# Circuitscape/Circuitscape.jl

Measured on NVIDIA H100. Metric: pair_solves_per_sec, higher is better.
Workload: dtype f64

## Files before the change

### circuitscape_b200/csrc/cs_b200.cu

```cuda
#include "../../include/cs_b200.h"

#include <cuda_runtime.h>

#include <algorithm>
#include <chrono>
#include <cmath>
#include <cstdarg>
#include <cstdio>
#include <cstdlib>
#include <cstring>
#include <limits>
#include <string>
#include <vector>

#include "amg_host.hpp"
#include "win_host.hpp"
#include "kernels.cuh"
#include "raster_assembly.cuh"
#include "setup_device.hpp"

using namespace csb;

namespace {

thread_local std::string g_create_error;

struct GraphSlot {
  cudaGraphExec_t exec = nullptr;
  int chunk = 0;
  int64_t kernels = 0, spmms = 0;
  cudaGraphExec_t loop_exec = nullptr;
  int64_t loop_kernels = 0, loop_spmms = 0;
};

}

struct DevCsr {
  int* rowptr = nullptr;
  int* colidx = nullptr;
  void* vals = nullptr;
  int* bstart = nullptr;
  int nblocks = 0;
  int nrows = 0;
  int64_t nnz = 0;
  int lpr = 1;
  WinMeta* win_meta = nullptr;
  unsigned char* blob = nullptr;
  int has_dinv = 0;
// ... 10 lines not shown
struct DevLevel {
  int64_t n = 0, n_pad = 0;
  DevCsr A, P, R;
  void* dinv = nullptr;
  double omega = 2.0 / 3.0;
  void *x = nullptr, *b = nullptr, *t = nullptr, *y = nullptr;
};

struct cs_b200_handle {
  int device = 0;
  int dtype = CS_B200_F64;
  int64_t n = 0, n_pad = 0, nnz = 0;
  int* d_rowptr = nullptr;
  int* d_colidx = nullptr;
  void* d_vals = nullptr;
  bool owns_matrix = true;
  void* d_vals0 = nullptr;
  void* d_dinv = nullptr;
  int* d_bstart = nullptr;
  int nblocks = 0;
  int ktmax = 8;
  void *X = nullptr, *R = nullptr, *P = nullptr, *AP = nullptr, *B = nullptr, *stage = nullptr;
  void* Z = nullptr;
  DevCsr A0;
  std::vector<DevLevel> lv;
  double* d_pinv = nullptr;
  double amg_opc = 0.0;
  bool amg = false;
  bool mixed = false;
  std::vector<DevLevel> lv32;
  void *R32 = nullptr, *X32 = nullptr, *T32 = nullptr, *Z32 = nullptr;
  void *d_cum = nullptr, *d_max = nullptr;
  PanelCtl* d_ctl = nullptr;
  PanelCtl* h_ctl = nullptr;
  double* d_partials = nullptr;
  float* d_flush = nullptr;
  size_t flush_elems = 0;
  cudaStream_t stream = nullptr;
  cudaEvent_t ev0 = nullptr, ev1 = nullptr, ev2 = nullptr, ev3 = nullptr;
  long long* d_sp_rows = nullptr;
  double* d_sp_vals = nullptr;
  int* d_sp_ptr = nullptr;
  size_t sp_cap = 0;
  long long* d_probe = nullptr;
  void* d_probe_out = nullptr;
  size_t probe_cap = 0;
  cudaStream_t s_in = nullptr, s_out = nullptr;
  void* io_in[2] = {nullptr, nullptr};
  void* io_out[2] = {nullptr, nullptr};
  cudaEvent_t ev_in[2] = {nullptr, nullptr}, ev_used[2] = {nullptr, nullptr};
  cudaEvent_t ev_ready[2] = {nullptr, nullptr}, ev_out[2] = {nullptr, nullptr};
  int num_sms = 132;
  int grid_spmm = 132, grid_ew = 132;
  cs_b200_opts opts{};
  cs_b200_stats stats{};
  GraphSlot graphs[4];
  bool rg_on = false;
  int* d_rg_seg = nullptr;
  int* d_rg_rows = nullptr;
  size_t rg_cap = 0;
  GraphSlot rgraphs[4];
  int profile = 0;
  std::vector<cudaEvent_t> prof_ev;
  size_t prof_used = 0;
  double prof_ms = 0.0;
  double prof_bytes = 0.0;
  int64_t prof_launches = 0;
  std::vector<int> prof_slot;
  std::vector<double> prof_pair_bytes;
  double prof_slot_ms[16] = {}, prof_slot_bytes[16] = {};
  int64_t prof_slot_launches[16] = {};
  std::string err;
  size_t esize() const { return dtype == CS_B200_F64 ? 8 : 4; }
};

namespace {

struct Tick {
  bool on = std::getenv("CS_B200_VERBOSE") != nullptr;
  std::chrono::steady_clock::time_point t0 = std::chrono::steady_clock::now();
  void operator()(const char* what) {
    if (!on) return;
    const auto t1 = std::chrono::steady_clock::now();
    std::fprintf(stderr, "[cs_b200 setup] %-28s %8.1f ms\n", what,
                 std::chrono::duration<double, std::milli>(t1 - t0).count());
    t0 = t1;
  }
};

int set_err(cs_b200_handle* h, int code, const char* fmt, ...) {
  char buf[1024];
  va_list ap;
  va_start(ap, fmt);
  vsnprintf(buf, sizeof buf, fmt, ap);
// ... 525 lines not shown
  rc = build_operators<T>(h, hp, job, dseed);
  if (rc) return rc;
  return cs_b200_reset_currents(h);
}

template <typename T>
int build_operators(cs_b200_handle* h, const csb_dev::HostPattern& hp, csb_dev::SeedJob* job,
                    const csb_dev::DeviceSeed* dseed) {
  int rc = CS_B200_OK;
  k_dinv<T><<<std::min<int64_t>((h->n_pad + 255) / 256, 4096), 256, 0, h->stream>>>(
      (int)h->n, (int)h->n_pad, h->d_rowptr, h->d_colidx, (const T*)h->d_vals, (T*)h->d_dinv);
  const bool want_win = h->opts.window >= 0 && (h->opts.window > 0 || h->n >= 20000) && (win_mask() & 1);
  const bool want_amg = h->opts.precond == CS_B200_PRECOND_AMG;
  Tick tick;
  if (want_win || h->opts.stencil > 0) {
    rc = device_stencil<T>(h, h->A0);
    if (!rc && !h->A0.dia && want_win) rc = device_windows<T>(h, h->A0, h->n_pad, (const T*)h->d_dinv);
    if (rc) { csb_dev::seed_discard(job); return rc; }
    tick(h->A0.dia ? "finest operator: stencil form" : "finest operator: windows");
  }
  if (want_amg) {
    rc = setup_amg_device<T>(h, hp, job, dseed);
    if (rc) return rc;
  } else {
    csb_dev::seed_discard(job);
  }
  Tick tick1;
  csb_dev::trim_pool(h->device);
  tick1("scratch pool released");
  return CS_B200_OK;
}

int common_create(cs_b200_handle* h, const cs_b200_opts* opts) {
  if (opts) h->opts = *opts;
  if (h->opts.panel_width == 0) h->opts.panel_width = 8;
  if (h->opts.check_every <= 0) h->opts.check_every = 16;
  if (h->opts.resid_gate <= 0) h->opts.resid_gate = 1e-4;
  if (h->opts.use_graph == 0) h->opts.use_graph = 1;
  const int pw = h->opts.panel_width;
  if (pw != 1 && pw != 2 && pw != 4 && pw != 8)
    return set_err(h, CS_B200_ERR_ARG, "panel_width must be 1, 2, 4 or 8 (got %d)", pw);
  h->ktmax = pw;
  if (h->opts.precond != CS_B200_PRECOND_JACOBI && h->opts.precond != CS_B200_PRECOND_AMG)
    return set_err(h, CS_B200_ERR_UNSUPPORTED, "unknown preconditioner %d", h->opts.precond);
  int ndev = 0;
  cudaError_t e = cudaGetDeviceCount(&ndev);
// ... 84 lines not shown
    }
  } else if (m.lpr == 4 && KT * 4 <= 32) {
    k_spmm<T, KT, MODE, (KT * 4 <= 32 ? 4 : 1)><<<grid, NT, 0, h->stream>>>(view<T>(m), X, Y, ep);
  } else {
    k_spmm<T, KT, MODE, 1><<<grid, NT, 0, h->stream>>>(view<T>(m), X, Y, ep);
  }
  if (prof) cudaEventRecord(e1, h->stream);
  h->stats.kernel_launches++;
  if (timed) h->stats.spmm_launches++;
}

template <typename T, int KT, int MODE>
void launch_spmm(cs_b200_handle* h, const T* X, T* Y, const T* B) {
  launch_spmm_on<T, KT, MODE>(h, h->A0, X, Y, B, (const T*)h->d_dinv, 0.0, true);
}

void harvest_profile(cs_b200_handle* h) {
  for (size_t i = 0; i + 1 < h->prof_used; i += 2) {
    float ms = 0;
    if (cudaEventElapsedTime(&ms, h->prof_ev[i], h->prof_ev[i + 1]) == cudaSuccess) {
      h->prof_ms += ms;
      h->prof_launches++;
      if (i / 2 < h->prof_slot.size()) {
        const int sl = h->prof_slot[i / 2] & 15;
        h->prof_slot_ms[sl] += ms;
        h->prof_slot_bytes[sl] += h->prof_pair_bytes[i / 2];
        h->prof_slot_launches[sl]++;
      }
    }
  }
  h->prof_used = 0;
  h->prof_slot.clear();
  h->prof_pair_bytes.clear();
}

template <typename T, int KT>
int ew_grid(cs_b200_handle* h) {
  const size_t nelem = (size_t)h->n_pad * KT;
  const size_t per = (size_t)NT * Vec<T>::N;
  return (int)std::min<size_t>(h->grid_ew, (nelem + per - 1) / per);
}

template <typename T, int KT>
int ew_grid_n(cs_b200_handle* h, int64_t n_pad) {
  const size_t nelem = (size_t)n_pad * KT;
  const size_t per = (size_t)NT * Vec<T>::N;
  return (int)std::max<size_t>(1, std::min<size_t>(h->grid_ew, (nelem + per - 1) / per));
// ... 143 lines not shown
  k_seg_set<T, KT><<<2 * KT, NT, 0, h->stream>>>((T*)panel, h->d_rg_seg, h->d_rg_rows, set_b_only, v);
  h->stats.kernel_launches++;
}

template <typename T, int KT>
void mask_z(cs_b200_handle* h) {
  if (!h->rg_on) return;
  if (h->mixed) launch_seg_set<float, KT>(h, h->Z32, 0, 0.0f);
  else launch_seg_set<T, KT>(h, h->Z, 0, T(0));
}

inline GraphSlot& graph_slot(cs_b200_handle* h, int kt) {
  return (h->rg_on ? h->rgraphs : h->graphs)[kt_index(kt)];
}

void drop_graphs(GraphSlot* slots) {
  for (int i = 0; i < 4; ++i) {
    if (slots[i].exec) cudaGraphExecDestroy(slots[i].exec);
    if (slots[i].loop_exec) cudaGraphExecDestroy(slots[i].loop_exec);
    slots[i] = GraphSlot{};
  }
}

template <typename T, int KT>
void launch_iteration(cs_b200_handle* h) {
  const size_t nelem = (size_t)h->n_pad * KT;
  const int g = ew_grid<T, KT>(h);
  launch_spmm<T, KT, SP_CG>(h, (const T*)h->P, (T*)h->AP, nullptr);
  if (h->rg_on) launch_seg_set<T, KT>(h, h->AP, 0, T(0));
  if (!h->amg) {
    k_cg_update_r<T, KT><<<g, NT, 0, h->stream>>>(nelem, (const T*)h->AP, (const T*)h->d_dinv,
                                                  (T*)h->R, h->d_ctl, h->d_partials);
    k_cg_update_xp<T, KT><<<g, NT, 0, h->stream>>>(nelem, (const T*)h->R, (const T*)h->d_dinv,
                                                   (T*)h->X, (T*)h->P, h->d_ctl);
    h->stats.kernel_launches += 2;
  } else {
    if (h->mixed) {
      k_cg_update_r0<T, KT, float><<<g, NT, 0, h->stream>>>(nelem, (const T*)h->AP, (const T*)h->d_dinv,
                                                            (T)h->lv[0].omega, (T*)h->R,
                                                            implicit_x0(h->lv32[0]) ? nullptr : (float*)h->X32,
                                                            (float*)h->R32, h->d_ctl);
      launch_vcycle<T, KT>(h, true);
      mask_z<T, KT>(h);
      k_cg_update_xp2<T, KT, float><<<g, NT, 0, h->stream>>>(nelem, (const float*)h->Z32, (T*)h->X, (T*)h->P,
                                                             h->d_ctl);
    } else {
      k_cg_update_r0<T, KT, T><<<g, NT, 0, h->stream>>>(nelem, (const T*)h->AP, (const T*)h->d_dinv,
                                                        (T)h->lv[0].omega, (T*)h->R,
                                                        implicit_x0(h->lv[0]) ? nullptr : (T*)h->stage, nullptr,
                                                        h->d_ctl);
      launch_vcycle<T, KT>(h, true);
      mask_z<T, KT>(h);
      k_cg_update_xp2<T, KT, T><<<g, NT, 0, h->stream>>>(nelem, (const T*)h->Z, (T*)h->X, (T*)h->P, h->d_ctl);
    }
    h->stats.kernel_launches += 2;
  }
}

template <typename T, int KT>
int run_chunk(cs_b200_handle* h, int chunk) {
  GraphSlot& gs = graph_slot(h, KT);
  if (h->opts.use_graph > 0 && !h->profile) {
    if (!gs.exec || gs.chunk != chunk) {
      if (gs.exec) cudaGraphExecDestroy(gs.exec);
      gs.exec = nullptr;
      cudaGraph_t graph;
      const int64_t kl = h->stats.kernel_launches, sl = h->stats.spmm_launches;
      CK(h, cudaStreamBeginCapture(h->stream, cudaStreamCaptureModeThreadLocal));
      for (int i = 0; i < chunk; ++i) launch_iteration<T, KT>(h);
      CK(h, cudaStreamEndCapture(h->stream, &graph));
      gs.kernels = h->stats.kernel_launches - kl;
      gs.spmms = h->stats.spmm_launches - sl;
      h->stats.kernel_launches = kl;
      h->stats.spmm_launches = sl;
      CK(h, cudaGraphInstantiate(&gs.exec, graph, 0));
      cudaGraphDestroy(graph);
      gs.chunk = chunk;
    }
    CK(h, cudaGraphLaunch(gs.exec, h->stream));
// ... 41 lines not shown
    CK(h, cudaGraphInstantiate(&gs.loop_exec, graph, 0));
    cudaGraphDestroy(graph);
  }
  CK(h, cudaGraphLaunch(gs.loop_exec, h->stream));
  return CS_B200_OK;
}

template <typename T, int KT>
int solve_panel(cs_b200_handle* h, double rtol, int64_t itmax) {
  const size_t nelem = (size_t)h->n_pad * KT;
  const double atol = h->opts.atol > 0 ? h->opts.atol
                      : h->opts.atol < 0 ? 0.0
                      : std::sqrt(std::numeric_limits<double>::epsilon());
  const int g = ew_grid<T, KT>(h);
  const int imax = (int)std::min<int64_t>(itmax, std::numeric_limits<int>::max() - 1);
  CK(h, cudaEventRecord(h->ev2, h->stream));
  if (!h->amg) {
    k_set_stall<<<1, 1, 0, h->stream>>>(h->d_ctl, 2000);
    k_cg_init<T, KT><<<g, NT, 0, h->stream>>>(nelem, (const T*)h->B, (const T*)h->d_dinv, (T*)h->X,
                                              (T*)h->R, (T*)h->P, h->d_ctl, h->d_partials, rtol, atol,
                                              imax);
    h->stats.kernel_launches++;
  } else {
    CK(h, cudaMemsetAsync(h->X, 0, nelem * sizeof(T), h->stream));
    CK(h, cudaMemsetAsync(h->P, 0, nelem * sizeof(T), h->stream));
    CK(h, cudaMemcpyAsync(h->R, h->B, nelem * sizeof(T), cudaMemcpyDeviceToDevice, h->stream));
    k_set_ctl<<<1, 1, 0, h->stream>>>(h->d_ctl, rtol, atol, imax, 40);
    if (h->mixed) {
      k_convert<T, float><<<g, NT, 0, h->stream>>>(nelem, (const T*)h->R, (float*)h->R32);
      launch_vcycle<T, KT>(h, false);
      mask_z<T, KT>(h);
      k_cg_update_xp2<T, KT, float><<<g, NT, 0, h->stream>>>(nelem, (const float*)h->Z32, (T*)h->X, (T*)h->P,
                                                             h->d_ctl);
      h->stats.kernel_launches++;
    } else {
      launch_vcycle<T, KT>(h, false);
      mask_z<T, KT>(h);
      k_cg_update_xp2<T, KT, T><<<g, NT, 0, h->stream>>>(nelem, (const T*)h->Z, (T*)h->X, (T*)h->P, h->d_ctl);
    }
    h->stats.kernel_launches += 2;
  }
  CK(h, cudaGetLastError());
  const int chunk = h->amg ? std::min(h->opts.check_every, 4) : h->opts.check_every;
  const bool device_loop = h->opts.use_graph == 1 && !h->profile;
  if (device_loop) {
    int rc = run_loop<T, KT>(h);
    if (rc) return rc;
  }
  for (;;) {
    CK(h, cudaMemcpyAsync(h->h_ctl, h->d_ctl, sizeof(PanelCtl), cudaMemcpyDeviceToHost, h->stream));
    CK(h, cudaStreamSynchronize(h->stream));
    if (h->profile) harvest_profile(h);
    if (device_loop) {
      GraphSlot& gs = graph_slot(h, KT);
      h->stats.kernel_launches += 1 + gs.loop_kernels * h->h_ctl->iter;
      h->stats.spmm_launches += gs.loop_spmms * h->h_ctl->iter;
      break;
    }
    if (h->h_ctl->nactive == 0) break;
    int rc = run_chunk<T, KT>(h, chunk);
    if (rc) return rc;
  }
  if (h->rg_on) {
    launch_spmm<T, KT, SP_RES>(h, (const T*)h->X, (T*)h->AP, (const T*)h->B);
    launch_seg_set<T, KT>(h, h->AP, 0, T(0));
    k_resnorm<T, KT><<<g, NT, 0, h->stream>>>(nelem, (size_t)h->n * KT, (const T*)h->AP, (const T*)h->B, h->d_ctl, h->d_partials);
    h->stats.kernel_launches++;
  } else {
    launch_spmm<T, KT, 2>(h, (const T*)h->X, (T*)h->AP, (const T*)h->B);
  }
  CK(h, cudaGetLastError());
  CK(h, cudaEventRecord(h->ev3, h->stream));
  CK(h, cudaMemcpyAsync(h->h_ctl, h->d_ctl, sizeof(PanelCtl), cudaMemcpyDeviceToHost, h->stream));
  CK(h, cudaStreamSynchronize(h->stream));
  if (h->profile) harvest_profile(h);
  float ms = 0;
  CK(h, cudaEventElapsedTime(&ms, h->ev2, h->ev3));
  h->stats.kernel_ms += ms;
  return CS_B200_OK;
}

int gather_panel_status(cs_b200_handle* h, int kt, int64_t c0, int64_t* iters, double* relres,
                        int64_t itmax, bool* any_fail, bool* any_maxit, std::string* msg) {
  for (int c = 0; c < kt; ++c) {
    const PanelCtl& ct = *h->h_ctl;
// ... 728 lines not shown
  k_set_ctl<<<1, 1, 0, h->stream>>>(h->d_ctl, 0.0, 0.0, 1, 40);
  const T* zp = (const T*)h->Z;
  if (h->mixed) {
    k_convert<T, float><<<g, NT, 0, h->stream>>>(nelem, (const T*)h->R, (float*)h->R32);
    launch_vcycle<T, KT>(h, false);
    k_convert<float, T><<<g, NT, 0, h->stream>>>(nelem, (const float*)h->Z32, (T*)h->X);
    zp = (const T*)h->X;
  } else {
    launch_vcycle<T, KT>(h, false);
  }
  k_panel_to_cm<T, KT><<<tg, 256, 0, h->stream>>>((int)h->n, (size_t)h->n, zp, (T*)h->stage, h->d_ctl, 0);
  CK(h, cudaGetLastError());
  CK(h, cudaMemcpyAsync(z, h->stage, bytes, cudaMemcpyDeviceToHost, h->stream));
  CK(h, cudaMemcpyAsync(h->h_ctl, h->d_ctl, sizeof(PanelCtl), cudaMemcpyDeviceToHost, h->stream));
  CK(h, cudaStreamSynchronize(h->stream));
  if (rz)
    for (int c = 0; c < KT; ++c) rz[c] = h->h_ctl->rho0[c];
  return CS_B200_OK;
}


extern "C" {

int cs_b200_version(void) { return 1004; }

const char* cs_b200_last_error(const cs_b200_handle* h) {
  return h ? h->err.c_str() : g_create_error.c_str();
}

int cs_b200_create(int64_t n, int64_t nnz, const void* rowptr, const void* colidx,
                   const void* vals, int index_bits, int index_base, int dtype, int device,
                   const cs_b200_opts* opts, cs_b200_handle** out) {
  if (!out) return set_err(nullptr, CS_B200_ERR_ARG, "out is NULL");
  *out = nullptr;
  if (n <= 0 || nnz < 0 || !rowptr || (nnz > 0 && (!colidx || !vals)))
    return set_err(nullptr, CS_B200_ERR_ARG, "bad matrix arguments (n=%lld nnz=%lld)",
                   (long long)n, (long long)nnz);
  if ((index_bits != 32 && index_bits != 64) || (index_base != 0 && index_base != 1) ||
      (dtype != CS_B200_F32 && dtype != CS_B200_F64))
    return set_err(nullptr, CS_B200_ERR_ARG, "bad index_bits/index_base/dtype");
  if (nnz >= (int64_t)1 << 31 || n >= (int64_t)1 << 31)
    return set_err(nullptr, CS_B200_ERR_UNSUPPORTED,
                   "n and nnz must be < 2^31 (device indices are int32)");
  cs_b200_handle* h = new cs_b200_handle();
  h->n = n; h->nnz = nnz; h->dtype = dtype; h->device = device;
  int rc = common_create(h, opts);
  if (rc) { g_create_error = h->err; cs_b200_destroy(h); return rc; }
// ... 373 lines not shown
                                   : build_operators<float>(h, none, nullptr, nullptr);
  if (rc) return rc;
  cudaEventRecord(h->ev1, h->stream);
  cudaEventSynchronize(h->ev1);
  float ms = 0;
  cudaEventElapsedTime(&ms, h->ev0, h->ev1);
  h->stats.setup_ms = ms;
  return CS_B200_OK;
}

int cs_b200_get_dims(const cs_b200_handle* h, int64_t* n, int64_t* nnz) {
  if (!h) return CS_B200_ERR_ARG;
  if (n) *n = h->n;
  if (nnz) *nnz = h->nnz;
  return CS_B200_OK;
}

void cs_b200_destroy(cs_b200_handle* h) {
  if (!h) return;
  cudaSetDevice(h->device);
  teardown_operators(h);
  if (h->owns_matrix) { cudaFree(h->d_rowptr); cudaFree(h->d_colidx); cudaFree(h->d_vals); }
  cudaFree(h->d_vals0);
  void* bufs[] = {h->d_dinv, h->d_bstart, h->X, h->R, h->P, h->AP, h->B, h->stage,
                  h->d_cum, h->d_max, h->d_ctl, h->d_partials, h->d_flush};
  for (void* b : bufs) if (b) cudaFree(b);
  if (h->h_ctl) cudaFreeHost(h->h_ctl);
  cudaFree(h->d_sp_rows); cudaFree(h->d_sp_vals); cudaFree(h->d_sp_ptr);
  cudaFree(h->d_probe); cudaFree(h->d_probe_out);
  cudaFree(h->d_rg_seg); cudaFree(h->d_rg_rows);
  for (int i = 0; i < 2; ++i) {
    cudaFree(h->io_in[i]); cudaFree(h->io_out[i]);
    cudaEvent_t evs[] = {h->ev_in[i], h->ev_used[i], h->ev_ready[i], h->ev_out[i]};
    for (cudaEvent_t e : evs) if (e) cudaEventDestroy(e);
  }
  if (h->s_in) cudaStreamDestroy(h->s_in);
  if (h->s_out) cudaStreamDestroy(h->s_out);
  for (cudaEvent_t e : h->prof_ev) cudaEventDestroy(e);
  if (h->ev0) cudaEventDestroy(h->ev0);
  if (h->ev1) cudaEventDestroy(h->ev1);
  if (h->ev2) cudaEventDestroy(h->ev2);
  if (h->ev3) cudaEventDestroy(h->ev3);
  if (h->stream) cudaStreamDestroy(h->stream);
  delete h;
}

int cs_b200_reset_currents(cs_b200_handle* h) {
// ... 24 lines not shown
  if (d_cum) *d_cum = h->d_cum;
  if (d_max) *d_max = h->d_max;
  return CS_B200_OK;
}

int cs_b200_stream(cs_b200_handle* h, void** stream) {
  if (!h || !stream) return CS_B200_ERR_ARG;
  *stream = (void*)h->stream;
  return CS_B200_OK;
}

int cs_b200_profile_spmm(cs_b200_handle* h, int enable, double* total_ms, int64_t* launches) {
  if (!h) return CS_B200_ERR_ARG;
  if (total_ms) *total_ms = h->prof_ms;
  if (launches) *launches = h->prof_launches;
  if (enable >= 0) {
    h->profile = enable ? 1 : 0;
    h->prof_ms = 0.0;
    h->prof_launches = 0;
    h->prof_used = 0;
    h->prof_bytes = 0.0;
    h->prof_slot.clear();
    h->prof_pair_bytes.clear();
    for (int i = 0; i < 16; ++i) { h->prof_slot_ms[i] = 0.0; h->prof_slot_bytes[i] = 0.0; h->prof_slot_launches[i] = 0; }
  }
  return CS_B200_OK;
}

int cs_b200_profile_classes(cs_b200_handle* h, double* ms16, double* bytes16, int64_t* launches16) {
  if (!h) return CS_B200_ERR_ARG;
  for (int i = 0; i < 16; ++i) {
    if (ms16) ms16[i] = h->prof_slot_ms[i];
    if (bytes16) bytes16[i] = h->prof_slot_bytes[i];
    if (launches16) launches16[i] = h->prof_slot_launches[i];
  }
  return CS_B200_OK;
}

int cs_b200_profile_bytes(cs_b200_handle* h, double* algorithmic_bytes) {
  if (!h || !algorithmic_bytes) return CS_B200_ERR_ARG;
  *algorithmic_bytes = h->prof_bytes;
  return CS_B200_OK;
}

int cs_b200_get_stats(const cs_b200_handle* h, cs_b200_stats* out) {
  if (!h || !out) return CS_B200_ERR_ARG;
  *out = h->stats;
  return CS_B200_OK;
}

int cs_b200_spmv(cs_b200_handle* h, const void* x, void* y, int reps, double* ms_per_rep) {
  if (!h || !x || !y || reps < 1) return set_err(h, CS_B200_ERR_ARG, "bad spmv arguments");
  begin_call(h);
  const size_t bytes = (size_t)h->n * h->esize();
  CK(h, cudaMemcpyAsync(h->X, x, bytes, cudaMemcpyHostToDevice, h->stream));
  CK(h, cudaEventRecord(h->ev2, h->stream));
  for (int r = 0; r < reps; ++r) {
// ... 564 lines not shown
```

### circuitscape_b200/csrc/kernels.cuh

```cuda
#pragma once
#include <cuda_runtime.h>
#include <stdint.h>

namespace csb {

constexpr int NT = 256;
constexpr int NWARP = NT / 32;
constexpr int NNZ_CAP = 2304;
constexpr int MAXKT = 8;

struct PanelCtl {
  double rho[MAXKT];
  double pap[MAXKT];
  double alpha[MAXKT];
  double beta[MAXKT];
  double tol[MAXKT];
  double rho0[MAXKT];
  double resid[MAXKT];
  double bnorm[MAXKT];
  double xsrc[MAXKT];
  double xdst[MAXKT];
  double maxpos[MAXKT];
  double maxneg[MAXKT];
  double weight[MAXKT];
  long long src[MAXKT];
  long long dst[MAXKT];
  int active[MAXKT];
  int iters[MAXKT];
  int iter;
  int itmax;
  int nactive;
  unsigned int ticket;
  int init;
  double rtol, atol;
  double best[MAXKT];
  int stall[MAXKT];
  int stall_limit;
  int stalled[MAXKT];
};

__device__ __forceinline__ int ld_stream(const int* p) {
  int v;
  asm volatile("ld.global.nc.L1::no_allocate.s32 %0, [%1];" : "=r"(v) : "l"(p));
  return v;
}
__device__ __forceinline__ float ld_stream(const float* p) {
  float v;
  asm volatile("ld.global.nc.L1::no_allocate.f32 %0, [%1];" : "=f"(v) : "l"(p));
  return v;
}
__device__ __forceinline__ double ld_stream(const double* p) {
  double v;
  asm volatile("ld.global.nc.L1::no_allocate.f64 %0, [%1];" : "=d"(v) : "l"(p));
  return v;
}

template <int KT> struct Log2 { static constexpr int v = 1 + Log2<KT / 2>::v; };
template <> struct Log2<1> { static constexpr int v = 0; };

template <typename T> struct Vec;
template <> struct Vec<double> { using type = double2; static constexpr int N = 2; };
// ... 86 lines not shown
  }
  if (o < NOUT && l == 0) out[o] = s_tree[tid];
  if (tid == 0) *ticket = 0u;
  __syncthreads();
  return true;
}

template <int KT>
__device__ __forceinline__ void cg_after_precond(PanelCtl* ctl, const double* rho_new) {
  const int c = threadIdx.x;
  const int init = ctl->init;
  const int it = ctl->iter + 1;
  __syncthreads();
  if (c < KT) {
    const double rn = fabs(rho_new[c]);
    if (init) {
      const double tol = ctl->atol + ctl->rtol * sqrt(rn);
      ctl->rho[c] = rn;
      ctl->rho0[c] = rn;
      ctl->tol[c] = tol;
      ctl->active[c] = (rn > 0.0 && sqrt(rn) > tol && ctl->itmax > 0) ? 1 : 0;
      ctl->iters[c] = 0;
      ctl->alpha[c] = 0.0;
      ctl->beta[c] = 0.0;
      ctl->best[c] = rn;
      ctl->stall[c] = 0;
      ctl->stalled[c] = 0;
    } else if (ctl->active[c]) {
      const double ro = ctl->rho[c];
      ctl->beta[c] = ro > 0.0 ? rn / ro : 0.0;
      ctl->rho[c] = rn;
      ctl->iters[c] = it;
      if (rn < 0.81 * ctl->best[c]) { ctl->best[c] = rn; ctl->stall[c] = 0; }
      else if (++ctl->stall[c] >= ctl->stall_limit && ctl->stall_limit > 0) { ctl->stalled[c] = 1; ctl->active[c] = 0; }
      if (!(sqrt(rn) > ctl->tol[c]) || it >= ctl->itmax) ctl->active[c] = 0;
    } else {
      ctl->beta[c] = 0.0;
    }
  }
  __syncthreads();
  if (c == 0) {
    int na = 0;
    for (int k = 0; k < KT; ++k) na += ctl->active[k];
    ctl->nactive = na;
    ctl->iter = init ? 0 : it;
    ctl->init = 0;
// ... 251 lines not shown
                                 MODE == SP_JACOBI_DOT || MODE == SP_ADD);
  static constexpr int al(int x) { return (x + 127) / 128 * 128; }
  static constexpr int XW = al((WIDE ? W_WCAP_WIDE : W_WCAP) * KT * (int)sizeof(T));
  static constexpr int BW = NEEDB ? al((W_RB + 8) * KT * (int)sizeof(T)) : 0;
  static constexpr int VW = al(W_NNZ * ((int)sizeof(T) + 2) + (W_RB + 8) * (2 + (int)sizeof(T)));
  static constexpr int OFF_X = 0;
  static constexpr int OFF_B = OFF_X + XW;
  static constexpr int OFF_V = OFF_B + BW;
  static constexpr int STAGE = OFF_V + VW;
  static constexpr int NSTAGE = (W_SMEM_BUDGET / STAGE) >= 6 ? 6 : (W_SMEM_BUDGET / STAGE);
  static constexpr int TOTAL = NSTAGE * STAGE;
};

constexpr int WC = 512;
constexpr int WTT = WC + 32;

__device__ __forceinline__ void mbar_arrive(unsigned long long* bar) {
  asm volatile("mbarrier.arrive.shared::cta.b64 _, [%0];" ::"r"(smem_u32(bar)) : "memory");
}
__device__ __forceinline__ void consumer_sync() {
  asm volatile("bar.sync 1, %0;" ::"r"(WC) : "memory");
}

template <typename T, int N>
__device__ __forceinline__ void ldvec(const T* p, T (&v)[N]) {
  constexpr int BYTES = N * (int)sizeof(T);
  if constexpr (BYTES >= 16) {
    constexpr int PER = 16 / (int)sizeof(T);
#pragma unroll
    for (int k = 0; k < N / PER; ++k) {
      const uint4 t = *reinterpret_cast<const uint4*>(p + k * PER);
      const T* q = reinterpret_cast<const T*>(&t);
#pragma unroll
      for (int i = 0; i < PER; ++i) v[k * PER + i] = q[i];
    }
  } else if constexpr (BYTES == 8) {
    const uint2 t = *reinterpret_cast<const uint2*>(p);
    const T* q = reinterpret_cast<const T*>(&t);
#pragma unroll
    for (int i = 0; i < N; ++i) v[i] = q[i];
  } else {
    v[0] = p[0];
  }
}
template <typename T, int N>
__device__ __forceinline__ void stvec(T* p, const T (&v)[N]) {
  constexpr int BYTES = N * (int)sizeof(T);
  if constexpr (BYTES >= 16) {
    constexpr int PER = 16 / (int)sizeof(T);
#pragma unroll
    for (int k = 0; k < N / PER; ++k) {
      uint4 t;
      T* q = reinterpret_cast<T*>(&t);
#pragma unroll
      for (int i = 0; i < PER; ++i) q[i] = v[k * PER + i];
      *reinterpret_cast<uint4*>(p + k * PER) = t;
    }
  } else if constexpr (BYTES == 8) {
    uint2 t;
    T* q = reinterpret_cast<T*>(&t);
#pragma unroll
    for (int i = 0; i < N; ++i) q[i] = v[i];
    *reinterpret_cast<uint2*>(p) = t;
  } else {
    p[0] = v[0];
// ... 412 lines not shown
      }
    }
  } else if (MODE == SP_RESNORM) {
    CSB_REDUCE_SMEM(2, KT)
    double v[2][CPT];
#pragma unroll
    for (int i = 0; i < CPT; ++i) { v[0][i] = dot0[i]; v[1][i] = dot1[i]; }
    if (grid_reduce<KT, CPT, 2, false>(v, ep.partials, &ep.ctl->ticket, s_warp, s_tree, s_out)) {
      if (tid < KT) {
        ep.ctl->resid[tid] = s_out[tid];
        ep.ctl->bnorm[tid] = s_out[KT + tid];
      }
    }
  } else if (MODE == SP_JACOBI_DOT) {
    CSB_REDUCE_SMEM(1, KT)
    double v[1][CPT];
#pragma unroll
    for (int i = 0; i < CPT; ++i) v[0][i] = dot0[i];
    if (grid_reduce<KT, CPT, 1, false>(v, ep.partials, &ep.ctl->ticket, s_warp, s_tree, s_out))
      cg_after_precond<KT>(ep.ctl, s_out);
  }
}

constexpr int PJ_RING = 4;
constexpr int PJ_MINB_F32 = 3;
constexpr int PJ_MINB_F64 = 2;

template <typename T> struct CsrP {
  const int* rowptr;
  const int* colidx;
  const T* vals;
  const int* ell_col;
  const T* ell_val;
  size_t ell_ld;
};

template <typename T, int KT> struct PjShape {
  static constexpr int V16 = 16 / (int)sizeof(T);
  static constexpr int CPT = KT < V16 ? KT : V16;
  static constexpr int CG = KT / CPT;
  static constexpr int RH = NT / CG;
  static constexpr int RPS = RH - 2;
  static constexpr bool VSMEM = sizeof(T) == 4;
  static constexpr int SMEM = (PJ_RING * RH * KT + 2 * NT * CPT + 2 * NT + (VSMEM ? 2 * 9 * RH : 0)) * (int)sizeof(T);
};

// ... 367 lines not shown
  const size_t stride = (size_t)gridDim.x * NT * VEC;
  T al[VEC], be[VEC];
#pragma unroll
  for (int i = 0; i < VEC; ++i) {
    al[i] = (T)ctl->alpha[(e0 + i) % KT];
    be[i] = (T)ctl->beta[(e0 + i) % KT];
  }
  for (size_t e = e0; e < nelem; e += stride) {
    TV z[VEC];
    T p[VEC], x[VEC];
    ldvec<TV, VEC>(Z + e, z);
    vload(P + e, p);
    vload(X + e, x);
#pragma unroll
    for (int i = 0; i < VEC; ++i) {
      x[i] += al[i] * p[i];
      p[i] = (T)z[i] + be[i] * p[i];
    }
    vstore(X + e, x);
    vstore(P + e, p);
  }
}

template <typename TI, typename TO>
__global__ void __launch_bounds__(NT)
k_convert(size_t nelem, const TI* __restrict__ in, TO* __restrict__ out) {
  for (size_t e = (size_t)blockIdx.x * NT + threadIdx.x; e < nelem; e += (size_t)gridDim.x * NT)
    out[e] = (TO)in[e];
}

template <typename T, int KT>
__global__ void __launch_bounds__(NT)
k_jacobi0(size_t nelem, const T* __restrict__ B, const T* __restrict__ dinv, T omega,
          T* __restrict__ X) {
  constexpr int VEC = Vec<T>::N;
  constexpr int L = Log2<KT>::v;
  const size_t stride = (size_t)gridDim.x * NT * VEC;
  for (size_t e = ((size_t)blockIdx.x * NT + threadIdx.x) * VEC; e < nelem; e += stride) {
    T b[VEC], x[VEC];
    vload(B + e, b);
#pragma unroll
    for (int i = 0; i < VEC; ++i) x[i] = omega * dinv[(e + i) >> L] * b[i];
    vstore(X + e, x);
  }
}

// ... 418 lines not shown
```

### circuitscape_b200/solver.py

```python
from __future__ import annotations

import ctypes as C
from dataclasses import dataclass

import numpy as np
import scipy.sparse as sp

from . import _lib

CUDAB200 = ["cuda", "gpu", "b200", "cg+jacobi+cuda", "cg+amg+cuda"]


@dataclass
class CUDASolver:
    bs: int = 1000
    precision: str = "double"
    device: int = 0
    rtol: float = 1e-6
    itmax: int = 100_000
    precond: str = "amg"
    panel_width: int = 8
    check_every: int = 16
    use_graph: object = True
    window: str = "auto"
# ... 164 lines not shown
        return self

    def __exit__(self, *a):
        self.close()

    def stats(self):
        st = _lib.Stats()
        self._lib.cs_b200_get_stats(self._h, C.byref(st))
        return st.as_dict()

    def stream_ptr(self):
        p = C.c_void_p()
        _lib.check(self._lib, self._h, self._lib.cs_b200_stream(self._h, C.byref(p)))
        return p.value or 0

    def profile_spmm(self, enable):
        ms, cnt = C.c_double(), C.c_int64()
        _lib.check(self._lib, self._h,
                   self._lib.cs_b200_profile_spmm(self._h, -1 if enable is None else int(bool(enable)),
                                                  C.byref(ms), C.byref(cnt)))
        return ms.value, cnt.value

    def profile_classes(self):
        ms = np.zeros(16)
        by = np.zeros(16)
        ln = np.zeros(16, dtype=np.int64)
        _lib.check(self._lib, self._h, self._lib.cs_b200_profile_classes(self._h, _lib._ptr(ms), _lib._ptr(by), _lib._ptr(ln)))
        names = ["plain", "cg", "residual_gate", "residual", "jacobi", "jacobi_dot", "prolong_add", "prolong_jacobi_fused"]
        return {f"{names[i // 2]}_{'f32' if i % 2 else 'f64'}": (float(ms[i]), float(by[i]), int(ln[i]))
                for i in range(16) if ln[i]}

    def profile_bytes(self):
        b = C.c_double()
        _lib.check(self._lib, self._h, self._lib.cs_b200_profile_bytes(self._h, C.byref(b)))
        return b.value

    def spmv(self, x, reps=1):
        x = np.ascontiguousarray(x, dtype=self.dtype)
        y = np.empty_like(x)
        ms = C.c_double()
        rc = self._lib.cs_b200_spmv(self._h, _lib._ptr(x), _lib._ptr(y), reps, C.byref(ms))
        _lib.check(self._lib, self._h, rc)
        return y, ms.value

    def spmm(self, X):
        X = np.asfortranarray(X, dtype=self.dtype)
        Y = np.empty_like(X, order="F")
        rc = self._lib.cs_b200_spmm(self._h, X.shape[1], _lib._ptr(X), _lib._ptr(Y))
        _lib.check(self._lib, self._h, rc)
        return Y

    def apply_precond(self, R):
        R = np.asarray(R, dtype=self.dtype)
# ... 222 lines not shown
```

### include/cs_b200.h

```cpp
#ifndef CS_B200_H
#define CS_B200_H

#include <stdint.h>

#ifdef __cplusplus
extern "C" {
#endif

typedef struct cs_b200_handle cs_b200_handle;

enum cs_b200_status {
  CS_B200_OK = 0,
  CS_B200_ERR_ARG = -1,
  CS_B200_ERR_CUDA = -2,
  CS_B200_ERR_RESIDUAL = -3,
  CS_B200_ERR_MAXITER = -4,
  CS_B200_ERR_UNSUPPORTED = -5
};

enum cs_b200_dtype { CS_B200_F32 = 0, CS_B200_F64 = 1 };

enum cs_b200_precond {
  CS_B200_PRECOND_JACOBI = 0,
  CS_B200_PRECOND_AMG = 1
// ... 108 lines not shown
int cs_b200_profile_spmm(cs_b200_handle* h, int enable, double* total_ms, int64_t* launches);

int cs_b200_profile_bytes(cs_b200_handle* h, double* algorithmic_bytes);

typedef struct cs_b200_comm cs_b200_comm;

int cs_b200_comm_unique_id(void* id128);
int cs_b200_comm_init(int device, int rank, int nranks, const void* id128, cs_b200_comm** out);
void cs_b200_comm_destroy(cs_b200_comm* c);
const char* cs_b200_comm_last_error(const cs_b200_comm* c);

int cs_b200_create_bcast(cs_b200_comm* c, int root, int64_t n, int64_t nnz, const void* rowptr,
                         const void* colidx, const void* vals, int index_bits, int index_base,
                         int dtype, const cs_b200_opts* opts, cs_b200_handle** out);

int cs_b200_comm_reduce_currents(cs_b200_comm* c, cs_b200_handle* h);

int cs_b200_comm_gather_pairs(cs_b200_comm* c, int64_t k_total, const int64_t* my_idx,
                              int64_t k_mine, const double* my_R, double* R_all);

int cs_b200_comm_max_double(cs_b200_comm* c, double* v, int count);
int cs_b200_comm_barrier(cs_b200_comm* c);

int cs_b200_profile_classes(cs_b200_handle* h, double* ms16, double* bytes16, int64_t* launches16);

int cs_b200_version(void);

#ifdef __cplusplus
}
#endif
#endif
```

### profiles/run_iteration_breakdown.py

```python
#!/usr/bin/env python
import argparse
import ctypes as C
import json
import os
import re
import subprocess
import sys
from collections import defaultdict

sys.path.insert(0, os.path.dirname(os.path.dirname(os.path.abspath(__file__))))
import numpy as np

PEAK_GBS = 3350.0
KT = 8


def card():
    try:
        out = subprocess.run(["nvidia-smi", "--query-gpu=name,power.limit", "--format=csv,noheader"],
                             capture_output=True, text=True, timeout=30).stdout.strip().splitlines()
        name, pl = [s.strip() for s in out[0].split(",")]
        return {"name": name, "power_limit": pl}
    except Exception as e:
        return {"name": None, "power_limit": None, "error": str(e)}
# ... 24 lines not shown
            depth += 1
        elif ch == ">":
            depth -= 1
        elif ch == "(" and depth == 0:
            cut = i
            break
    return name[:cut].replace(" ", "")


def finest_bytes(levels, prolong_form):
    n = levels[0]["A"][0]
    n1 = levels[1]["A"][0] if len(levels) > 1 else 0
    nnz_r = levels[0]["R"][2] if levels[0]["R"] else 0
    d64, d32 = 8 * KT, 4 * KT
    rps = 256 // 2 - 2
    if prolong_form == "tile":
        halo = (130 * 10) / (128 * 8)
        prol = n * (halo * (d32 + 4 + 32 + d32) + 9 * 4 + d32 + 4 + d32)
    else:
        halo = (rps + 2) / rps
        prol = n * (halo * (d32 + 4 + 32 + d32) + 9 * 4 + d32)
    return {
        "k_stencil<double,8,1>": n * (9 * 8 + d64 + d64),
        "k_cg_update_r0<double,8,float>": n * (d64 + 8 + 2 * d64 + d32),
        "k_stencil<float,8,7>": n * (9 * 4 + d32 + 4 + d32),
        "k_spmm_win<float,8,0,*>#1": nnz_r * 6 + n1 * 2 + n * d32 + n1 * d32,
        "k_stencil_prolong_jacobi<float,8,5,*>": prol,
        "k_cg_update_xp2<double,8,float>": n * (d32 + 4 * d64),
    }, {"n": n, "n1": n1, "nnz_R0": nnz_r, "prolong_halo_factor": halo}


def match_bytes(key, table):
    for pat, b in table.items():
        base, _, occ = pat.partition("#")
        rx = "^" + re.escape(base).replace(r"\*", r"[^,>]+") + "$"
        name, _, slot = key.partition("#")
        if re.match(rx, name) and (not occ or (slot or "1").split("/")[0] == occ):
            return b
    return None


def main():
    ap = argparse.ArgumentParser()
    ap.add_argument("--rows", type=int, default=3163)
    ap.add_argument("--reps", type=int, default=20)
    ap.add_argument("--prolong-form", default="strip", choices=["strip", "tile"])
    ap.add_argument("--out", default="")
    a = ap.parse_args()

    import torch
    from torch.profiler import ProfilerActivity, profile
    import circuitscape_b200 as cb
    from circuitscape_b200 import graph
    if not torch.cuda.is_available():
        raise SystemExit("needs a CUDA device")
    L, _ = graph.synthetic_raster_laplacian(a.rows, a.rows, seed=42)
    with cb.construct_cholesky_factor(L, cb.CUDASolver()) as f:
        levels = level_dims(f)
        f.bench_cg_iter(KT, reps=5)
        ms_iter = f.bench_cg_iter(KT, reps=a.reps)
        torch.cuda.synchronize()
        with profile(activities=[ProfilerActivity.CUDA]) as prof:
            f.bench_cg_iter(KT, reps=a.reps)
            torch.cuda.synchronize()
    evs = [e for e in prof.events() if e.device_type.name == "CUDA" and "memcpy" not in e.name.lower()
           and "memset" not in e.name.lower()]
    evs.sort(key=lambda e: e.time_range.start)
    starts = [i for i, e in enumerate(evs) if short(e.name).startswith("k_stencil<double,8,1>")
              or short(e.name).startswith("k_spmm_win<double,8,1,")]
    iters = [evs[starts[j]:starts[j + 1]] for j in range(len(starts) - 1)]
    iters = iters[3:] if len(iters) > a.reps else iters
    if len(starts) > 1:
        last = evs[starts[-1]:]
        iters.append(last[:len(iters[0])] if iters else last)
    agg = defaultdict(lambda: [0, 0.0])
    for it in iters:
        names = [short(e.name) for e in it]
        tot = defaultdict(int)
        for nm in names:
            tot[nm] += 1
        seen = defaultdict(int)
        for e, nm in zip(it, names):
            seen[nm] += 1
            key = nm if tot[nm] == 1 else f"{nm}#{seen[nm]}/{tot[nm]}"
            agg[key][0] += 1
            agg[key][1] += e.time_range.elapsed_us()
    niter = max(1, len(iters))
    table, shape = finest_bytes(levels, a.prolong_form)
    sum_us = sum(v[1] for v in agg.values()) / niter
    rows = {}
    for key, (cnt, us) in sorted(agg.items(), key=lambda kv: -kv[1][1]):
        avg = us / cnt
# ... 20 lines not shown
```

Before: 119.6.

## Fuse P update and deferred X update into stencil SpMM for AMG-CG

When AMG preconditioning and the stencil (DIA) form are both active, the separate x/p update kernel is removed. The stencil kernel now forms p = z + beta*p on the fly from the Z panel and the previous P, applies A to it, and writes the new P to a second, double-buffered P panel. X updates are deferred and applied two steps at a time using a ring of saved alphas, plus a final tail kernel after the loop. This drops one kernel launch and one full panel read/write pass per iteration. In exchange the stencil kernel does redundant neighbour P/Z loads, uses more registers, and needs an extra P buffer.

Result: faster. 124.8, median of 6 (+4.3%).

```diff
diff --git a/circuitscape_b200/csrc/cs_b200.cu b/circuitscape_b200/csrc/cs_b200.cu
--- a/circuitscape_b200/csrc/cs_b200.cu
+++ b/circuitscape_b200/csrc/cs_b200.cu
@@ -24,6 +24,9 @@
 namespace {
 
 thread_local std::string g_create_error;
+
+constexpr int PROF_CLASSES = 18;
+constexpr int PROF_CGF = 8;
 
 struct GraphSlot {
   cudaGraphExec_t exec = nullptr;
@@ -80,6 +83,7 @@
   int ktmax = 8;
   void *X = nullptr, *R = nullptr, *P = nullptr, *AP = nullptr, *B = nullptr, *stage = nullptr;
   void* Z = nullptr;
+  void* P2 = nullptr;
   DevCsr A0;
   std::vector<DevLevel> lv;
   double* d_pinv = nullptr;
@@ -126,8 +130,8 @@
   int64_t prof_launches = 0;
   std::vector<int> prof_slot;
   std::vector<double> prof_pair_bytes;
-  double prof_slot_ms[16] = {}, prof_slot_bytes[16] = {};
-  int64_t prof_slot_launches[16] = {};
+  double prof_slot_ms[PROF_CLASSES] = {}, prof_slot_bytes[PROF_CLASSES] = {};
+  int64_t prof_slot_launches[PROF_CLASSES] = {};
   std::string err;
   size_t esize() const { return dtype == CS_B200_F64 ? 8 : 4; }
 };
@@ -699,6 +703,12 @@
   if (want_amg) {
     rc = setup_amg_device<T>(h, hp, job, dseed);
     if (rc) return rc;
+    if (h->amg && h->A0.dia && !h->P2) {
+      const size_t pe = (size_t)h->n_pad * h->ktmax * sizeof(T);
+      cudaError_t e = cudaMalloc(&h->P2, pe);
+      if (e == cudaSuccess) e = cudaMemsetAsync(h->P2, 0, pe, h->stream);
+      if (e != cudaSuccess) return set_err(h, CS_B200_ERR_CUDA, "CUDA error %s (second p panel)", cudaGetErrorString(e));
+    }
   } else {
     csb_dev::seed_discard(job);
   }
@@ -829,7 +839,7 @@
       h->prof_ms += ms;
       h->prof_launches++;
       if (i / 2 < h->prof_slot.size()) {
-        const int sl = h->prof_slot[i / 2] & 15;
+        const int sl = h->prof_slot[i / 2];
         h->prof_slot_ms[sl] += ms;
         h->prof_slot_bytes[sl] += h->prof_pair_bytes[i / 2];
         h->prof_slot_launches[sl]++;
@@ -1019,11 +1029,52 @@
   }
 }
 
+inline bool fused_cg(const cs_b200_handle* h) {
+  static const bool off = std::getenv("CS_B200_NO_FUSED_CG") != nullptr;
+  return h->amg && h->A0.dia && h->P2 && !off;
+}
+
+template <typename T, int KT, typename TV>
+void launch_stencil_cg(cs_b200_handle* h, const TV* Z) {
+  const DevCsr& m = h->A0;
+  const DiaDev<T> a{(const T*)m.dia, m.dia_ld, m.nrows, m.dia_nr};
+  constexpr int V16 = 16 / (int)sizeof(T);
+  constexpr int CGn = KT / (KT < V16 ? KT : V16);
+  const int rpp = NT / CGn;
+  const long long ntiles = (long long)((m.dia_nr + rpp - 1) / rpp) *
+                           ((((long long)m.nrows + m.dia_nr - 1) / m.dia_nr + ST_TC - 1) / ST_TC);
+  const int sg = (int)std::max<long long>(1, std::min<long long>(h->grid_spmm, ntiles));
+  cudaEvent_t e0 = nullptr, e1 = nullptr;
+  if (h->profile) {
+    if (h->prof_used + 2 > h->prof_ev.size())
+      for (int i = 0; i < 2; ++i) { cudaEvent_t e; cudaEventCreate(&e); h->prof_ev.push_back(e); }
+    e0 = h->prof_ev[h->prof_used++];
+    e1 = h->prof_ev[h->prof_used++];
+    const double pe = (double)m.nrows * KT * sizeof(T);
+    const double fb = (double)m.nrows * 9 * sizeof(T) + (double)m.nrows * KT * sizeof(TV) + 3.0 * pe + 1.5 * pe;
+    h->prof_bytes += fb;
+    h->prof_slot.push_back(2 * PROF_CGF + (sizeof(T) == 4 ? 1 : 0));
+    h->prof_pair_bytes.push_back(fb);
+    cudaEventRecord(e0, h->stream);
+  }
+  k_stencil_cg<T, KT, TV><<<sg, NT, 0, h->stream>>>(a, Z, (T*)h->P2, (T*)h->P, (T*)h->X, (T*)h->AP, h->d_ctl,
+                                                     h->d_partials);
+  if (h->profile) cudaEventRecord(e1, h->stream);
+  h->stats.kernel_launches++;
+  h->stats.spmm_launches++;
+}
+
 template <typename T, int KT>
 void launch_iteration(cs_b200_handle* h) {
   const size_t nelem = (size_t)h->n_pad * KT;
   const int g = ew_grid<T, KT>(h);
-  launch_spmm<T, KT, SP_CG>(h, (const T*)h->P, (T*)h->AP, nullptr);
+  const bool fused = fused_cg(h);
+  if (fused) {
+    if (h->mixed) launch_stencil_cg<T, KT, float>(h, (const float*)h->Z32);
+    else launch_stencil_cg<T, KT, T>(h, (const T*)h->Z);
+  } else {
+    launch_spmm<T, KT, SP_CG>(h, (const T*)h->P, (T*)h->AP, nullptr);
+  }
   if (h->rg_on) launch_seg_set<T, KT>(h, h->AP, 0, T(0));
   if (!h->amg) {
     k_cg_update_r<T, KT><<<g, NT, 0, h->stream>>>(nelem, (const T*)h->AP, (const T*)h->d_dinv,
@@ -1039,8 +1090,9 @@
                                                             (float*)h->R32, h->d_ctl);
       launch_vcycle<T, KT>(h, true);
       mask_z<T, KT>(h);
-      k_cg_update_xp2<T, KT, float><<<g, NT, 0, h->stream>>>(nelem, (const float*)h->Z32, (T*)h->X, (T*)h->P,
-                                                             h->d_ctl);
+      if (!fused)
+        k_cg_update_xp2<T, KT, float><<<g, NT, 0, h->stream>>>(nelem, (const float*)h->Z32, (T*)h->X, (T*)h->P,
+                                                               h->d_ctl);
     } else {
       k_cg_update_r0<T, KT, T><<<g, NT, 0, h->stream>>>(nelem, (const T*)h->AP, (const T*)h->d_dinv,
                                                         (T)h->lv[0].omega, (T*)h->R,
@@ -1048,10 +1100,19 @@
                                                         h->d_ctl);
       launch_vcycle<T, KT>(h, true);
       mask_z<T, KT>(h);
-      k_cg_update_xp2<T, KT, T><<<g, NT, 0, h->stream>>>(nelem, (const T*)h->Z, (T*)h->X, (T*)h->P, h->d_ctl);
-    }
-    h->stats.kernel_launches += 2;
-  }
+      if (!fused)
+        k_cg_update_xp2<T, KT, T><<<g, NT, 0, h->stream>>>(nelem, (const T*)h->Z, (T*)h->X, (T*)h->P, h->d_ctl);
+    }
+    h->stats.kernel_launches += fused ? 1 : 2;
+  }
+}
+
+template <typename T, int KT>
+void finish_x(cs_b200_handle* h) {
+  if (!fused_cg(h)) return;
+  k_cg_x_tail<T, KT><<<ew_grid<T, KT>(h), NT, 0, h->stream>>>((size_t)h->n_pad * KT, (const T*)h->P2, (const T*)h->P,
+                                                             (T*)h->X, h->d_ctl);
+  h->stats.kernel_launches++;
 }
 
 template <typename T, int KT>
@@ -1139,6 +1200,7 @@
                                               imax);
     h->stats.kernel_launches++;
   } else {
+    const bool fused = fused_cg(h);
     CK(h, cudaMemsetAsync(h->X, 0, nelem * sizeof(T), h->stream));
     CK(h, cudaMemsetAsync(h->P, 0, nelem * sizeof(T), h->stream));
     CK(h, cudaMemcpyAsync(h->R, h->B, nelem * sizeof(T), cudaMemcpyDeviceToDevice, h->stream));
@@ -1147,15 +1209,17 @@
       k_convert<T, float><<<g, NT, 0, h->stream>>>(nelem, (const T*)h->R, (float*)h->R32);
       launch_vcycle<T, KT>(h, false);
       mask_z<T, KT>(h);
-      k_cg_update_xp2<T, KT, float><<<g, NT, 0, h->stream>>>(nelem, (const float*)h->Z32, (T*)h->X, (T*)h->P,
-                                                             h->d_ctl);
+      if (!fused)
+        k_cg_update_xp2<T, KT, float><<<g, NT, 0, h->stream>>>(nelem, (const float*)h->Z32, (T*)h->X, (T*)h->P,
+                                                               h->d_ctl);
       h->stats.kernel_launches++;
     } else {
       launch_vcycle<T, KT>(h, false);
       mask_z<T, KT>(h);
-      k_cg_update_xp2<T, KT, T><<<g, NT, 0, h->stream>>>(nelem, (const T*)h->Z, (T*)h->X, (T*)h->P, h->d_ctl);
-    }
-    h->stats.kernel_launches += 2;
+      if (!fused)
+        k_cg_update_xp2<T, KT, T><<<g, NT, 0, h->stream>>>(nelem, (const T*)h->Z, (T*)h->X, (T*)h->P, h->d_ctl);
+    }
+    h->stats.kernel_launches += fused ? 1 : 2;
   }
   CK(h, cudaGetLastError());
   const int chunk = h->amg ? std::min(h->opts.check_every, 4) : h->opts.check_every;
@@ -1178,6 +1242,7 @@
     int rc = run_chunk<T, KT>(h, chunk);
     if (rc) return rc;
   }
+  if (h->amg) finish_x<T, KT>(h);
   if (h->rg_on) {
     launch_spmm<T, KT, SP_RES>(h, (const T*)h->X, (T*)h->AP, (const T*)h->B);
     launch_seg_set<T, KT>(h, h->AP, 0, T(0));
@@ -1952,7 +2017,7 @@
 
 extern "C" {
 
-int cs_b200_version(void) { return 1004; }
+int cs_b200_version(void) { return 1005; }
 
 const char* cs_b200_last_error(const cs_b200_handle* h) {
   return h ? h->err.c_str() : g_create_error.c_str();
@@ -2372,7 +2437,7 @@
   teardown_operators(h);
   if (h->owns_matrix) { cudaFree(h->d_rowptr); cudaFree(h->d_colidx); cudaFree(h->d_vals); }
   cudaFree(h->d_vals0);
-  void* bufs[] = {h->d_dinv, h->d_bstart, h->X, h->R, h->P, h->AP, h->B, h->stage,
+  void* bufs[] = {h->d_dinv, h->d_bstart, h->X, h->R, h->P, h->P2, h->AP, h->B, h->stage,
                   h->d_cum, h->d_max, h->d_ctl, h->d_partials, h->d_flush};
   for (void* b : bufs) if (b) cudaFree(b);
   if (h->h_ctl) cudaFreeHost(h->h_ctl);
@@ -2443,17 +2508,17 @@
     h->prof_bytes = 0.0;
     h->prof_slot.clear();
     h->prof_pair_bytes.clear();
-    for (int i = 0; i < 16; ++i) { h->prof_slot_ms[i] = 0.0; h->prof_slot_bytes[i] = 0.0; h->prof_slot_launches[i] = 0; }
-  }
-  return CS_B200_OK;
-}
-
-int cs_b200_profile_classes(cs_b200_handle* h, double* ms16, double* bytes16, int64_t* launches16) {
+    for (int i = 0; i < PROF_CLASSES; ++i) { h->prof_slot_ms[i] = 0.0; h->prof_slot_bytes[i] = 0.0; h->prof_slot_launches[i] = 0; }
+  }
+  return CS_B200_OK;
+}
+
+int cs_b200_profile_classes(cs_b200_handle* h, double* ms18, double* bytes18, int64_t* launches18) {
   if (!h) return CS_B200_ERR_ARG;
-  for (int i = 0; i < 16; ++i) {
-    if (ms16) ms16[i] = h->prof_slot_ms[i];
-    if (bytes16) bytes16[i] = h->prof_slot_bytes[i];
-    if (launches16) launches16[i] = h->prof_slot_launches[i];
+  for (int i = 0; i < PROF_CLASSES; ++i) {
+    if (ms18) ms18[i] = h->prof_slot_ms[i];
+    if (bytes18) bytes18[i] = h->prof_slot_bytes[i];
+    if (launches18) launches18[i] = h->prof_slot_launches[i];
   }
   return CS_B200_OK;
 }
diff --git a/circuitscape_b200/csrc/kernels.cuh b/circuitscape_b200/csrc/kernels.cuh
--- a/circuitscape_b200/csrc/kernels.cuh
+++ b/circuitscape_b200/csrc/kernels.cuh
@@ -37,6 +37,7 @@
   int stall[MAXKT];
   int stall_limit;
   int stalled[MAXKT];
+  double alpha_ring[3][MAXKT];
 };
 
 __device__ __forceinline__ int ld_stream(const int* p) {
@@ -169,6 +170,7 @@
       ctl->active[c] = (rn > 0.0 && sqrt(rn) > tol && ctl->itmax > 0) ? 1 : 0;
       ctl->iters[c] = 0;
       ctl->alpha[c] = 0.0;
+      ctl->alpha_ring[0][c] = ctl->alpha_ring[1][c] = ctl->alpha_ring[2][c] = 0.0;
       ctl->beta[c] = 0.0;
       ctl->best[c] = rn;
       ctl->stall[c] = 0;
@@ -466,25 +468,27 @@
   asm volatile("bar.sync 1, %0;" ::"r"(WC) : "memory");
 }
 
-template <typename T, int N>
+template <typename T, int N, bool NC = false>
 __device__ __forceinline__ void ldvec(const T* p, T (&v)[N]) {
   constexpr int BYTES = N * (int)sizeof(T);
   if constexpr (BYTES >= 16) {
     constexpr int PER = 16 / (int)sizeof(T);
 #pragma unroll
     for (int k = 0; k < N / PER; ++k) {
-      const uint4 t = *reinterpret_cast<const uint4*>(p + k * PER);
+      const uint4* a = reinterpret_cast<const uint4*>(p + k * PER);
+      const uint4 t = NC ? __ldg(a) : *a;
       const T* q = reinterpret_cast<const T*>(&t);
 #pragma unroll
       for (int i = 0; i < PER; ++i) v[k * PER + i] = q[i];
     }
   } else if constexpr (BYTES == 8) {
-    const uint2 t = *reinterpret_cast<const uint2*>(p);
+    const uint2* a = reinterpret_cast<const uint2*>(p);
+    const uint2 t = NC ? __ldg(a) : *a;
     const T* q = reinterpret_cast<const T*>(&t);
 #pragma unroll
     for (int i = 0; i < N; ++i) v[i] = q[i];
   } else {
-    v[0] = p[0];
+    v[0] = NC ? __ldg(p) : p[0];
   }
 }
 template <typename T, int N>
@@ -943,6 +947,112 @@
   }
 }
 
+constexpr int CGF_MINB = 2;
+
+template <typename T, int KT, typename TV>
+__device__ __forceinline__ void stencil_cg_body(const DiaDev<T>& A, const TV* __restrict__ Z, const T* __restrict__ Pold,
+                                                T* __restrict__ Pd, T* __restrict__ X, T* __restrict__ Y,
+                                                PanelCtl* ctl, double* partials, int it) {
+  constexpr int V16 = 16 / (int)sizeof(T);
+  constexpr int CPT = KT < V16 ? KT : V16;
+  constexpr int CG = KT / CPT;
+  constexpr int RPP = NT / CG;
+  const int tid = threadIdx.x;
+  const int cg = tid % CG, rl = tid / CG, c0 = cg * CPT;
+  const int n = A.n, nr = A.nr;
+  const int ncol = (n + nr - 1) / nr;
+  const int nrc = (nr + RPP - 1) / RPP;
+  const int ntc = (ncol + ST_TC - 1) / ST_TC;
+  const long long ntiles = (long long)nrc * ntc;
+  const bool pair = it & 1;
+  T be[CPT], a1[CPT], a2[CPT];
+#pragma unroll
+  for (int i = 0; i < CPT; ++i) {
+    be[i] = (T)ctl->beta[c0 + i];
+    a1[i] = (T)ctl->alpha_ring[(it + 2) % 3][c0 + i];
+    a2[i] = (T)ctl->alpha_ring[(it + 1) % 3][c0 + i];
+  }
+  double dot0[CPT];
+#pragma unroll
+  for (int i = 0; i < CPT; ++i) dot0[i] = 0.0;
+
+  for (long long t = blockIdx.x; t < ntiles; t += gridDim.x) {
+    const int tc = (int)(t / nrc), rc = (int)(t % nrc);
+    const int r = rc * RPP + rl;
+    if (r >= nr) continue;
+    const int cend = min(ncol, (tc + 1) * ST_TC);
+    for (int c = tc * ST_TC; c < cend; ++c) {
+      const long long row_l = (long long)c * nr + r;
+      if (row_l >= n) break;
+      const int row = (int)row_l;
+      T v[9];
+#pragma unroll
+      for (int s = 0; s < 9; ++s) v[s] = __ldcs(A.vals + (size_t)s * A.ld + row);
+      TV zv[9][CPT];
+      T pv[9][CPT];
+#pragma unroll
+      for (int s = 0; s < 9; ++s) {
+        int j = row + (s / 3 - 1) * nr + (s % 3 - 1);
+        j = max(0, min(n - 1, j));
+        ldvec<TV, CPT>(Z + (size_t)j * KT + c0, zv[s]);
+        ldvec<T, CPT, true>(Pold + (size_t)j * KT + c0, pv[s]);
+      }
+      const size_t o = (size_t)row * KT + c0;
+      T xo[CPT], pd[CPT], po[CPT];
+      if (pair) {
+        ldvec<T, CPT>(X + o, xo);
+        ldvec<T, CPT>(Pd + o, pd);
+      }
+#pragma unroll
+      for (int i = 0; i < CPT; ++i) po[i] = pv[4][i];
+#pragma unroll
+      for (int s = 0; s < 9; ++s)
+#pragma unroll
+        for (int i = 0; i < CPT; ++i) pv[s][i] = (T)zv[s][i] + be[i] * pv[s][i];
+      T acc[CPT];
+#pragma unroll
+      for (int i = 0; i < CPT; ++i) acc[i] = T(0);
+#pragma unroll
+      for (int s = 0; s < 9; ++s)
+#pragma unroll
+        for (int i = 0; i < CPT; ++i) acc[i] += v[s] * pv[s][i];
+#pragma unroll
+      for (int i = 0; i < CPT; ++i) dot0[i] += (double)acc[i] * (double)pv[4][i];
+      stvec<T, CPT>(Y + o, acc);
+      stvec<T, CPT>(Pd + o, pv[4]);
+      if (pair) {
+#pragma unroll
+        for (int i = 0; i < CPT; ++i) {
+          xo[i] += a2[i] * pd[i];
+          xo[i] += a1[i] * po[i];
+        }
+        stvec<T, CPT>(X + o, xo);
+      }
+    }
+  }
+  CSB_REDUCE_SMEM(1, KT)
+  double v[1][CPT];
+#pragma unroll
+  for (int i = 0; i < CPT; ++i) v[0][i] = dot0[i];
+  if (grid_reduce<KT, CPT, 1, false>(v, partials, &ctl->ticket, s_warp, s_tree, s_out)) {
+    if (tid < KT) {
+      const double pap = s_out[tid];
+      const double al = (ctl->active[tid] && pap > 0.0) ? ctl->rho[tid] / pap : 0.0;
+      ctl->pap[tid] = pap;
+      ctl->alpha[tid] = al;
+      ctl->alpha_ring[it % 3][tid] = al;
+    }
+  }
+}
+
+template <typename T, int KT, typename TV>
+__global__ void __launch_bounds__(NT, CGF_MINB)
+k_stencil_cg(const DiaDev<T> A, const TV* __restrict__ Z, T* Pb0, T* Pb1, T* __restrict__ X, T* __restrict__ Y,
+             PanelCtl* ctl, double* partials) {
+  const int it = ctl->iter;
+  stencil_cg_body<T, KT, TV>(A, Z, (it & 1) ? Pb0 : Pb1, (it & 1) ? Pb1 : Pb0, X, Y, ctl, partials, it);
+}
+
 constexpr int PJ_RING = 4;
 constexpr int PJ_MINB_F32 = 3;
 constexpr int PJ_MINB_F64 = 2;
@@ -1356,6 +1466,38 @@
   }
 }
 
+template <typename T, int KT>
+__global__ void __launch_bounds__(NT)
+k_cg_x_tail(size_t nelem, const T* __restrict__ Pb0, const T* __restrict__ Pb1, T* __restrict__ X,
+            const PanelCtl* ctl) {
+  constexpr int VEC = Vec<T>::N;
+  const int K = ctl->iter;
+  const bool two = K & 1;
+  const T* p2 = (K & 1) ? Pb1 : Pb0;
+  const T* p1 = (K & 1) ? Pb0 : Pb1;
+  const size_t e0 = ((size_t)blockIdx.x * NT + threadIdx.x) * VEC;
+  const size_t stride = (size_t)gridDim.x * NT * VEC;
+  T a1[VEC], a2[VEC];
+#pragma unroll
+  for (int i = 0; i < VEC; ++i) {
+    a1[i] = (T)ctl->alpha_ring[(K + 2) % 3][(e0 + i) % KT];
+    a2[i] = (T)ctl->alpha_ring[(K + 1) % 3][(e0 + i) % KT];
+  }
+  for (size_t e = e0; e < nelem; e += stride) {
+    T x[VEC], q1[VEC], q2[VEC];
+    vload(X + e, x);
+    vload(p1 + e, q1);
+    if (two) {
+      vload(p2 + e, q2);
+#pragma unroll
+      for (int i = 0; i < VEC; ++i) x[i] += a2[i] * q2[i];
+    }
+#pragma unroll
+    for (int i = 0; i < VEC; ++i) x[i] += a1[i] * q1[i];
+    vstore(X + e, x);
+  }
+}
+
 template <typename TI, typename TO>
 __global__ void __launch_bounds__(NT)
 k_convert(size_t nelem, const TI* __restrict__ in, TO* __restrict__ out) {
diff --git a/circuitscape_b200/solver.py b/circuitscape_b200/solver.py
--- a/circuitscape_b200/solver.py
+++ b/circuitscape_b200/solver.py
@@ -210,13 +210,14 @@
         return ms.value, cnt.value
 
     def profile_classes(self):
-        ms = np.zeros(16)
-        by = np.zeros(16)
-        ln = np.zeros(16, dtype=np.int64)
+        names = ["plain", "cg", "residual_gate", "residual", "jacobi", "jacobi_dot", "prolong_add", "prolong_jacobi_fused",
+                 "cg_step_fused"]
+        ms = np.zeros(2 * len(names))
+        by = np.zeros(2 * len(names))
+        ln = np.zeros(2 * len(names), dtype=np.int64)
         _lib.check(self._lib, self._h, self._lib.cs_b200_profile_classes(self._h, _lib._ptr(ms), _lib._ptr(by), _lib._ptr(ln)))
-        names = ["plain", "cg", "residual_gate", "residual", "jacobi", "jacobi_dot", "prolong_add", "prolong_jacobi_fused"]
         return {f"{names[i // 2]}_{'f32' if i % 2 else 'f64'}": (float(ms[i]), float(by[i]), int(ln[i]))
-                for i in range(16) if ln[i]}
+                for i in range(2 * len(names)) if ln[i]}
 
     def profile_bytes(self):
         b = C.c_double()
diff --git a/include/cs_b200.h b/include/cs_b200.h
--- a/include/cs_b200.h
+++ b/include/cs_b200.h
@@ -154,7 +154,7 @@
 int cs_b200_comm_max_double(cs_b200_comm* c, double* v, int count);
 int cs_b200_comm_barrier(cs_b200_comm* c);
 
-int cs_b200_profile_classes(cs_b200_handle* h, double* ms16, double* bytes16, int64_t* launches16);
+int cs_b200_profile_classes(cs_b200_handle* h, double* ms18, double* bytes18, int64_t* launches18);
 
 int cs_b200_version(void);
 
diff --git a/profiles/run_iteration_breakdown.py b/profiles/run_iteration_breakdown.py
--- a/profiles/run_iteration_breakdown.py
+++ b/profiles/run_iteration_breakdown.py
@@ -70,6 +70,7 @@
         prol = n * (halo * (d32 + 4 + 32 + d32) + 9 * 4 + d32)
     return {
         "k_stencil<double,8,1>": n * (9 * 8 + d64 + d64),
+        "k_stencil_cg<double,8,float>": n * (9 * 8 + d32 + 3 * d64 + 1.5 * d64),
         "k_cg_update_r0<double,8,float>": n * (d64 + 8 + 2 * d64 + d32),
         "k_stencil<float,8,7>": n * (9 * 4 + d32 + 4 + d32),
         "k_spmm_win<float,8,0,*>#1": nnz_r * 6 + n1 * 2 + n * d32 + n1 * d32,
@@ -114,8 +115,8 @@
     evs = [e for e in prof.events() if e.device_type.name == "CUDA" and "memcpy" not in e.name.lower()
            and "memset" not in e.name.lower()]
     evs.sort(key=lambda e: e.time_range.start)
-    starts = [i for i, e in enumerate(evs) if short(e.name).startswith("k_stencil<double,8,1>")
-              or short(e.name).startswith("k_spmm_win<double,8,1,")]
+    starts = [i for i, e in enumerate(evs) if short(e.name).startswith(("k_stencil<double,8,1>", "k_stencil_cg<double,8,",
+                                                                        "k_spmm_win<double,8,1,"))]
     iters = [evs[starts[j]:starts[j + 1]] for j in range(len(starts) - 1)]
     iters = iters[3:] if len(iters) > a.reps else iters
     if len(starts) > 1:
```
